# showlab/EgoVLP

Hardware: NVIDIA H100
Metric: clips/sec, 16-frame TimeSformer-B + DistilBERT + EgoNCE training step (higher is better)
Workload: dtype bf16

## Files before the change

### egovlp_b200/csrc/attention.cu

```cuda
#include <stdlib.h>

#include "common.cuh"
#include "egovlp_b200.h"

namespace egovlp {

bool space_attn_wgmma_supported(int N);
int space_attn_fwd_wgmma(const void* qkv, void* out, float* lse, float* cls_part, int B, int T, int N, int H,
                         cudaStream_t st);

namespace {

constexpr int HD = 64;
constexpr int ROW_BYTES = 128;
constexpr float LOG2E = 1.4426950408889634f;

struct Geom {
  int B, H, T, N, S, D;
  int mode;
  int PG;
  int G;
  int NP;
  int NPAD;
  int gsize;
};

__device__ __forceinline__ int row_token(const Geom& G, int g, int r) {
  if (r == G.NP) return 0;
  if (r > G.NP) return -1;
  if (G.mode == 1) return 1 + g * G.N + r;
  const int j = r / G.T, f = r - j * G.T, n = g * G.PG + j;
  return n < G.N ? 1 + f * G.N + n : -1;
}

template <int RT>
__device__ __forceinline__ int row_token_x(const Geom& G, int g, int r, int sh) {
  if (RT == 0) return row_token(G, g, r);
  if (r == G.NP) return 0;
  if (r > G.NP) return -1;
  if (RT == 1) return 1 + g * G.N + r;
  const int n = g * G.PG + (r >> sh);
  return n < G.N ? 1 + (r & ((1 << sh) - 1)) * G.N + n : -1;
}

struct Smem {
  uint32_t q, k, v, dout;
  short* gid;
  float* lse;
  float* delta;
  uint32_t stage;
  uint32_t bar;
};

__device__ __forceinline__ bool pair_valid(int gq, int gk, bool first_group) {
  if (gq >= 0) return gk == gq || gk == -2;
  if (gq == -2) return gk >= 0 || (gk == -2 && first_group);
  return false;
}

__device__ __forceinline__ void tile_window(const Geom& G, int r0, int& lo, int& hi) {
  if (r0 <= G.NP && G.NP < r0 + 16) { lo = 0; hi = G.NP; return; }
  if (r0 > G.NP) { lo = 0; hi = 0; return; }
  lo = (r0 / G.gsize) * G.gsize;
  hi = min(G.NP, ((r0 + 15) / G.gsize + 1) * G.gsize);
}
__device__ __forceinline__ bool span_active(const Geom& G, int lo, int hi, int c0, int width) {
  return (c0 < hi && c0 + width > lo) || (c0 <= G.NP && G.NP < c0 + width);
}

template <int RT = 0>
__device__ __forceinline__ void store_rows_bf16(const float (&acc)[8][4], float s0, float s1, uint32_t stage,
                                                uint8_t* stage_gen, bf16* dst, long long ld, int col0, const Geom& G,
                                                int b, int g, int r0, int lane, bool skip_cls, int sh = 0) {
  const int gq = lane >> 2, t = lane & 3;
#pragma unroll
  for (int j = 0; j < 8; ++j) {
    const uint32_t lo = pack_bf16x2(acc[j][0] * s0, acc[j][1] * s0), hi = pack_bf16x2(acc[j][2] * s1, acc[j][3] * s1);
    asm volatile("st.shared.b32 [%0], %1;" ::"r"(sw_addr(stage, gq, j) + t * 4), "r"(lo));
    asm volatile("st.shared.b32 [%0], %1;" ::"r"(sw_addr(stage, gq + 8, j) + t * 4), "r"(hi));
  }
  __syncwarp();
#pragma unroll
  for (int p = 0; p < 4; ++p) {
    const int rr = p * 4 + (lane >> 3), c = lane & 7;
    const int tok = row_token_x<RT>(G, g, r0 + rr, sh);
    if (tok > 0 || (tok == 0 && !skip_cls)) {
      const uint4 v = *reinterpret_cast<const uint4*>(stage_gen + (sw_addr(stage, rr, c) - stage));
      *reinterpret_cast<uint4*>(dst + ((long long)b * G.S + tok) * ld + col0 + c * 8) = v;
    }
  }
  __syncwarp();
}

template <int RT = 0>
__device__ __forceinline__ void store_frag_rows_bf16(const float (&acc)[8][4], float s, bf16* dst, long long ld, int col0,
                                                     const Geom& G, int b, int g, int r0, int lane, float s_hi = -1.f,
                                                     int sh = 0) {
  const float sB = s_hi >= 0.f ? s_hi : s;
  const int gq = lane >> 2, t = lane & 3;
  const int tok0 = row_token_x<RT>(G, g, r0 + gq, sh), tok1 = row_token_x<RT>(G, g, r0 + gq + 8, sh);
  bf16* p0 = dst + ((long long)b * G.S + tok0) * ld + col0 + 2 * t;
  bf16* p1 = dst + ((long long)b * G.S + tok1) * ld + col0 + 2 * t;
#pragma unroll
  for (int j = 0; j < 8; ++j) {
    if (tok0 > 0) *reinterpret_cast<uint32_t*>(p0 + 8 * j) = pack_bf16x2(acc[j][0] * s, acc[j][1] * s);
    if (tok1 > 0) *reinterpret_cast<uint32_t*>(p1 + 8 * j) = pack_bf16x2(acc[j][2] * sB, acc[j][3] * sB);
  }
}

__device__ __forceinline__ int tile_uniform_gid(const short* gid, int r0) {
  const int a = gid[r0], b = gid[r0 + 15];
  return (a >= 0 && a == b) ? a : -1;
}

__device__ __forceinline__ void decode_block(const Geom& G, int& b, int& h, int& g) {
  h = blockIdx.x % G.H;
  const int bg = blockIdx.x / G.H;
  g = bg % G.G;
  b = bg / G.G;
}

template <bool BWD, bool STAGE = !BWD, bool WAIT = true, bool GID = true>
__device__ __forceinline__ void load_group(const Geom& G, const CUtensorMap* tm_qkv, const CUtensorMap* tm_do,
                                           const bf16* qkv, const bf16* dout, int b, int h, int g, uint8_t* smem_gen,
                                           uint32_t smem_base, Smem& sm, int nwarps) {
  const int tile_bytes = G.NPAD * ROW_BYTES;
  sm.q = smem_base;
  sm.k = sm.q + tile_bytes;
  sm.v = sm.k + tile_bytes;
  sm.dout = sm.v + tile_bytes;
  uint32_t off = (BWD ? 4 : 3) * tile_bytes;
  sm.stage = smem_base + off;
  if (STAGE) off += nwarps * 16 * ROW_BYTES;
  sm.lse = reinterpret_cast<float*>(smem_gen + off);
  off += G.NPAD * 4;
  sm.delta = reinterpret_cast<float*>(smem_gen + off);
  off += G.NPAD * 4;
  sm.gid = reinterpret_cast<short*>(smem_gen + off);
  off += ((G.NPAD * 2 + 15) / 16) * 16;
  sm.bar = smem_base + off;

  const int tid = threadIdx.x;
  if (tid == 0) {
    mbar_init(sm.bar, 1);
    fence_mbar_init();
  }
  __syncthreads();
  const int ntiles = BWD ? 4 : 3;
  if (tid == 0) {
    const int rows = (G.mode == 1) ? G.N : G.T * G.PG;
    mbar_expect_tx(sm.bar, (uint32_t)(ntiles * rows * ROW_BYTES));
    const int f0 = (G.mode == 1) ? g : 0, n0 = (G.mode == 1) ? 0 : g * G.PG;
    tma_load_5d(sm.q, tm_qkv, sm.bar, 0, f0, n0, 0 * G.H + h, b);
    tma_load_5d(sm.k, tm_qkv, sm.bar, 0, f0, n0, 1 * G.H + h, b);
    tma_load_5d(sm.v, tm_qkv, sm.bar, 0, f0, n0, 2 * G.H + h, b);
    if (BWD) tma_load_5d(sm.dout, tm_do, sm.bar, 0, f0, n0, h, b);
  }
  const int pad_rows = G.NPAD - G.NP;
  for (int i = tid; i < pad_rows * 8; i += blockDim.x) {
    const int c = i & 7, rr = i >> 3;
#pragma unroll
    for (int which = 0; which < ntiles; ++which) {
      uint4 val = make_uint4(0, 0, 0, 0);
      if (rr == 0) {
        const bf16* src = (which < 3) ? qkv + (long long)b * G.S * 3 * G.D + which * G.D + h * HD
                                      : dout + (long long)b * G.S * G.D + h * HD;
        val = *reinterpret_cast<const uint4*>(src + c * 8);
      }
      *reinterpret_cast<uint4*>(smem_gen + (sw_addr(sm.q + which * tile_bytes, G.NP + rr, c) - smem_base)) = val;
    }
  }
  if (GID) {
    for (int r = tid; r < G.NPAD; r += blockDim.x) {
      short gid = -1;
      if (r == G.NP) gid = -2;
      else if (r < G.NP && row_token(G, g, r) > 0) gid = (short)(r / G.gsize);
      sm.gid[r] = gid;
    }
  }
  __syncthreads();
  if (WAIT) mbar_wait(sm.bar, 0);
}

template <int NWARPS, int MINB>
__global__ void __launch_bounds__(NWARPS * 32, MINB)
divided_attn_fwd_kernel(const __grid_constant__ CUtensorMap tm_qkv, const bf16* __restrict__ qkv,
                        bf16* __restrict__ out, float* __restrict__ lse_out, float* __restrict__ cls_part, Geom G) {
  extern __shared__ uint8_t smem_raw[];
  const uint32_t smem_base = (smem_u32(smem_raw) + 1023u) & ~1023u;
  uint8_t* smem_gen = smem_raw + (smem_base - smem_u32(smem_raw));
  int b, h, g;
  decode_block(G, b, h, g);
  Smem sm;
  load_group<false>(G, &tm_qkv, nullptr, qkv, nullptr, b, h, g, smem_gen, smem_base, sm, NWARPS);

  const int warp = threadIdx.x >> 5, lane = threadIdx.x & 31;
  const int gq = lane >> 2, t = lane & 3;
  const bool first_group = (g == 0);
  const int NT = G.NPAD / 8;
  const uint32_t stage = sm.stage + warp * 16 * ROW_BYTES;
  uint8_t* stage_gen = smem_gen + (stage - smem_base);

  for (int rt = warp; rt * 16 <= G.NP; rt += NWARPS) {
    const int r0 = rt * 16;
    int lo, hi;
    tile_window(G, r0, lo, hi);
    uint32_t qf[4][4];
#pragma unroll
    for (int kk = 0; kk < 4; ++kk) load_a_frag(sm.q, r0, kk, lane, qf[kk]);
    const int gid0 = sm.gid[r0 + gq], gid1 = sm.gid[r0 + gq + 8];
    const int ugid = tile_uniform_gid(sm.gid, r0);
    float m0 = -INFINITY, m1 = -INFINITY, l0 = 0.f, l1 = 0.f;
    float o[8][4];
#pragma unroll
    for (int j = 0; j < 8; ++j) { o[j][0] = o[j][1] = o[j][2] = o[j][3] = 0.f; }

    for (int c0 = 0; c0 < NT; c0 += 8) {
      if (!span_active(G, lo, hi, c0 * 8, 64)) continue;
      float s[8][4];
#pragma unroll
      for (int j = 0; j < 8; ++j) { s[j][0] = s[j][1] = s[j][2] = s[j][3] = 0.f; }
#pragma unroll
      for (int p = 0; p < 4; ++p) {
        const int n0 = (c0 + 2 * p) * 8;
        if (c0 + 2 * p < NT && span_active(G, lo, hi, n0, 16)) {
#pragma unroll
          for (int kk = 0; kk < 4; ++kk) {
            uint32_t bf[4];
            load_b_frag_nk(sm.k, n0, kk, lane, bf);
            mma_bf16(s[2 * p], qf[kk], bf[0], bf[1]);
            mma_bf16(s[2 * p + 1], qf[kk], bf[2], bf[3]);
          }
        }
      }
      float cm0 = -INFINITY, cm1 = -INFINITY;
#pragma unroll
      for (int j = 0; j < 8; ++j) {
        const int col = (c0 + j) * 8 + 2 * t;
        const bool inb = (c0 + j) < NT;
        const bool fast = inb && ugid >= 0 && sm.gid[(c0 + j) * 8] == ugid && sm.gid[(c0 + j) * 8 + 7] == ugid;
        if (!fast) {
          const int k0 = inb ? sm.gid[col] : -1, k1 = inb ? sm.gid[col + 1] : -1;
          s[j][0] = pair_valid(gid0, k0, first_group) ? s[j][0] : -INFINITY;
          s[j][1] = pair_valid(gid0, k1, first_group) ? s[j][1] : -INFINITY;
          s[j][2] = pair_valid(gid1, k0, first_group) ? s[j][2] : -INFINITY;
          s[j][3] = pair_valid(gid1, k1, first_group) ? s[j][3] : -INFINITY;
        }
        cm0 = fmaxf(cm0, fmaxf(s[j][0], s[j][1]));
        cm1 = fmaxf(cm1, fmaxf(s[j][2], s[j][3]));
      }
      cm0 = fmaxf(cm0, __shfl_xor_sync(0xffffffffu, cm0, 1)); cm0 = fmaxf(cm0, __shfl_xor_sync(0xffffffffu, cm0, 2));
      cm1 = fmaxf(cm1, __shfl_xor_sync(0xffffffffu, cm1, 1)); cm1 = fmaxf(cm1, __shfl_xor_sync(0xffffffffu, cm1, 2));
      const float mn0 = fmaxf(m0, cm0), mn1 = fmaxf(m1, cm1);
      const float ms0 = (mn0 == -INFINITY) ? 0.f : mn0, ms1 = (mn1 == -INFINITY) ? 0.f : mn1;
      const float a0 = exp2f((m0 - ms0) * LOG2E), a1 = exp2f((m1 - ms1) * LOG2E);
      m0 = mn0; m1 = mn1;
      l0 *= a0; l1 *= a1;
#pragma unroll
      for (int j = 0; j < 8; ++j) { o[j][0] *= a0; o[j][1] *= a0; o[j][2] *= a1; o[j][3] *= a1; }
      uint32_t pf[4][4];
#pragma unroll
      for (int j = 0; j < 8; ++j) {
        const float p0 = exp2f((s[j][0] - ms0) * LOG2E), p1 = exp2f((s[j][1] - ms0) * LOG2E);
        const float p2 = exp2f((s[j][2] - ms1) * LOG2E), p3 = exp2f((s[j][3] - ms1) * LOG2E);
        l0 += p0 + p1; l1 += p2 + p3;
        pf[j >> 1][(j & 1) * 2] = pack_bf16x2(p0, p1);
        pf[j >> 1][(j & 1) * 2 + 1] = pack_bf16x2(p2, p3);
      }
#pragma unroll
      for (int kk = 0; kk < 4; ++kk) {
        const int k0 = (c0 + 2 * kk) * 8;
        if (c0 + 2 * kk < NT && span_active(G, lo, hi, k0, 16)) {
#pragma unroll
// ... 448 lines not shown
#pragma unroll
    for (int dp = 0; dp < 4; ++dp) {
      uint32_t bf[4];
      ldsm_x4_t(vb + fo.a[dp], bf);
      mma_bf16(o[2 * dp], pf[p], bf[0], bf[1]);
      mma_bf16(o[2 * dp + 1], pf[p], bf[2], bf[3]);
    }
  }
}

template <bool TIME, int NWARPS, int MINB>
__global__ void __launch_bounds__(NWARPS * 32, MINB)
fast_attn_fwd_kernel(const __grid_constant__ CUtensorMap tm_qkv, const bf16* __restrict__ qkv, bf16* __restrict__ out,
                     float* __restrict__ lse_out, float* __restrict__ cls_part, Geom G, int sh) {
  extern __shared__ uint8_t smem_raw[];
  const uint32_t smem_base = (smem_u32(smem_raw) + 1023u) & ~1023u;
  uint8_t* smem_gen = smem_raw + (smem_base - smem_u32(smem_raw));
  int b, h, g;
  decode_block(G, b, h, g);
  Smem sm;
  load_group<false, !TIME, true, false>(G, &tm_qkv, nullptr, qkv, nullptr, b, h, g, smem_gen, smem_base, sm, NWARPS);
  constexpr int RT = TIME ? 2 : 1;

  const int warp = threadIdx.x >> 5, lane = threadIdx.x & 31;
  const int gq = lane >> 2, t = lane & 3;
  FastCtx c;
  c.NP = G.NP; c.NPAD = G.NPAD; c.sh = sh; c.first_group = (g == 0);
  c.valid_keys = TIME ? min(G.PG, G.N - g * G.PG) * G.T : G.NP;
  const FragOff fo = make_frag_off(lane);
  const uint32_t stage = sm.stage + warp * 16 * ROW_BYTES;
  uint8_t* stage_gen = smem_gen + (stage - smem_base);

  for (int it = warp;; it += NWARPS) {
    int r0, part;
    if (!work_item<TIME, NWARPS>(c, it, r0, part)) break;
    const int rowA = r0 + gq, rowB = rowA + 8;
    uint32_t qf[4][4];
#pragma unroll
    for (int kk = 0; kk < 4; ++kk) ldsm_x4(sm.q + r0 * ROW_BYTES + fo.a[kk], qf[kk]);
    float m0 = -INFINITY, m1 = -INFINITY, l0 = 0.f, l1 = 0.f;
    float o[8][4];
#pragma unroll
    for (int j = 0; j < 8; ++j) { o[j][0] = o[j][1] = o[j][2] = o[j][3] = 0.f; }
    Chunk ch;
#pragma unroll 1
    for (int ci = 0; get_chunk<TIME, NWARPS, 4>(c, G.T, r0, part, ci, ch); ++ci) {
      switch (ch.np) {
        case 4: fwd_chunk<TIME, 4>(c, sm, fo, ch, qf, rowA, rowB, t, m0, m1, l0, l1, o); break;
        case 3: fwd_chunk<TIME, 3>(c, sm, fo, ch, qf, rowA, rowB, t, m0, m1, l0, l1, o); break;
        case 2: fwd_chunk<TIME, 2>(c, sm, fo, ch, qf, rowA, rowB, t, m0, m1, l0, l1, o); break;
        default: fwd_chunk<TIME, 1>(c, sm, fo, ch, qf, rowA, rowB, t, m0, m1, l0, l1, o); break;
      }
    }
    l0 += __shfl_xor_sync(0xffffffffu, l0, 1); l0 += __shfl_xor_sync(0xffffffffu, l0, 2);
    l1 += __shfl_xor_sync(0xffffffffu, l1, 1); l1 += __shfl_xor_sync(0xffffffffu, l1, 2);
    {
      const int rc = c.NP - r0;
      if (rc >= 0 && rc < 16 && (rc & 7) == gq) {
        const bool hi_half = rc >= 8;
        constexpr int PARTS = TIME ? NWARPS : 1;
        float* dst = cls_part + ((((long long)(b * G.H + h)) * G.G + g) * PARTS + max(part, 0)) * 66;
#pragma unroll
        for (int j = 0; j < 8; ++j) {
          dst[j * 8 + 2 * t] = hi_half ? o[j][2] : o[j][0];
          dst[j * 8 + 2 * t + 1] = hi_half ? o[j][3] : o[j][1];
        }
        if (t == 0) { dst[64] = hi_half ? m1 : m0; dst[65] = hi_half ? l1 : l0; }
      }
    }
    if (part >= 0) continue;
    const float i0 = l0 > 0.f ? 1.f / l0 : 0.f, i1 = l1 > 0.f ? 1.f / l1 : 0.f;
    if (t == 0) {
      const int tok0 = row_token_x<RT>(G, g, rowA, sh), tok1 = row_token_x<RT>(G, g, rowB, sh);
      if (tok0 > 0) lse_out[((long long)(b * G.H + h)) * G.S + tok0] = m0 + logf(l0);
      if (tok1 > 0) lse_out[((long long)(b * G.H + h)) * G.S + tok1] = m1 + logf(l1);
    }
    if (TIME) store_frag_rows_bf16<RT>(o, i0, out, G.D, h * HD, G, b, g, r0, lane, i1, sh);
    else store_rows_bf16<RT>(o, i0, i1, stage, stage_gen, out, G.D, h * HD, G, b, g, r0, lane, true, sh);
  }
}

template <bool TIME, int NPR>
__device__ __forceinline__ void bwd_q_chunk(const FastCtx& c, const Smem& sm, const FragOff& fo, const Chunk& ch, int r0,
                                            int rowA, int rowB, int t, float ls0, float ls1, float de0, float de1,
                                            float (&dq)[8][4]) {
  float s[2 * NPR][4], dp[2 * NPR][4];
#pragma unroll
  for (int j = 0; j < 2 * NPR; ++j) { s[j][0] = s[j][1] = s[j][2] = s[j][3] = 0.f; dp[j][0] = dp[j][1] = dp[j][2] = dp[j][3] = 0.f; }
#pragma unroll
  for (int kk = 0; kk < 4; ++kk) {
    uint32_t aq[4], ad[4];
    ldsm_x4(sm.q + r0 * ROW_BYTES + fo.a[kk], aq);
    ldsm_x4(sm.dout + r0 * ROW_BYTES + fo.a[kk], ad);
#pragma unroll
    for (int p = 0; p < NPR; ++p) {
      uint32_t bf[4];
      ldsm_x4(sm.k + ch.base[p] * ROW_BYTES + fo.b[kk], bf);
      mma_bf16(s[2 * p], aq, bf[0], bf[1]);
      mma_bf16(s[2 * p + 1], aq, bf[2], bf[3]);
      ldsm_x4(sm.v + ch.base[p] * ROW_BYTES + fo.b[kk], bf);
      mma_bf16(dp[2 * p], ad, bf[0], bf[1]);
      mma_bf16(dp[2 * p + 1], ad, bf[2], bf[3]);
    }
  }
  uint32_t dsf[NPR][4];
  const f32x2 sc = pk2(LOG2E, LOG2E), nl0 = pk2(-ls0, -ls0), nl1 = pk2(-ls1, -ls1);
  const f32x2 nd0 = pk2(-de0, -de0), nd1 = pk2(-de1, -de1);
#pragma unroll
  for (int p = 0; p < NPR; ++p) {
    const bool masked = ch.mask & (1u << p);
#pragma unroll
    for (int jj = 0; jj < 2; ++jj) {
      const int j = 2 * p + jj, col = ch.base[p] + 8 * jj + 2 * t;
      if (masked) {
        if (TIME && ch.base[p] == c.NP && r0 < c.NP) {
          const bool kc = jj == 0 && t == 0;
          s[j][0] = kc ? s[j][0] : -INFINITY; s[j][1] = -INFINITY;
          s[j][2] = kc ? s[j][2] : -INFINITY; s[j][3] = -INFINITY;
        } else if (TIME && r0 >= c.NP && ch.base[p] < c.NP) {
          const bool cq = rowA == c.NP;
          s[j][0] = (cq && col < c.valid_keys) ? s[j][0] : -INFINITY;
          s[j][1] = (cq && col + 1 < c.valid_keys) ? s[j][1] : -INFINITY;
          s[j][2] = -INFINITY; s[j][3] = -INFINITY;
        } else {
          s[j][0] = fast_valid<TIME>(c, rowA, col) ? s[j][0] : -INFINITY;
          s[j][1] = fast_valid<TIME>(c, rowA, col + 1) ? s[j][1] : -INFINITY;
          s[j][2] = fast_valid<TIME>(c, rowB, col) ? s[j][2] : -INFINITY;
          s[j][3] = fast_valid<TIME>(c, rowB, col + 1) ? s[j][3] : -INFINITY;
        }
      }
      float e0, e1, e2, e3;
      up2(fma2(pk2(s[j][0], s[j][1]), sc, nl0), e0, e1);
      up2(fma2(pk2(s[j][2], s[j][3]), sc, nl1), e2, e3);
      float d0, d1, d2, d3;
      up2(mul2(pk2(exp2f(e0), exp2f(e1)), add2(pk2(dp[j][0], dp[j][1]), nd0)), d0, d1);
      up2(mul2(pk2(exp2f(e2), exp2f(e3)), add2(pk2(dp[j][2], dp[j][3]), nd1)), d2, d3);
      dsf[p][jj * 2] = pack_bf16x2(d0, d1);
      dsf[p][jj * 2 + 1] = pack_bf16x2(d2, d3);
    }
  }
#pragma unroll
  for (int p = 0; p < NPR; ++p) {
    const uint32_t kb = sm.k + ch.base[p] * ROW_BYTES;
#pragma unroll
    for (int dpi = 0; dpi < 4; ++dpi) {
      uint32_t bf[4];
      ldsm_x4_t(kb + fo.a[dpi], bf);
      mma_bf16(dq[2 * dpi], dsf[p], bf[0], bf[1]);
      mma_bf16(dq[2 * dpi + 1], dsf[p], bf[2], bf[3]);
    }
  }
}

template <bool TIME, int NPR>
__device__ __forceinline__ void bwd_k_chunk(const FastCtx& c, const Smem& sm, const FragOff& fo, const Chunk& ch, int k0r,
                                            int keyA, int keyB, int t, float (&dk)[8][4], float (&dv)[8][4]) {
  float st[2 * NPR][4], dpt[2 * NPR][4];
#pragma unroll
  for (int j = 0; j < 2 * NPR; ++j) { st[j][0] = st[j][1] = st[j][2] = st[j][3] = 0.f; dpt[j][0] = dpt[j][1] = dpt[j][2] = dpt[j][3] = 0.f; }
#pragma unroll
  for (int kk = 0; kk < 4; ++kk) {
    uint32_t ak[4], av[4];
    ldsm_x4(sm.k + k0r * ROW_BYTES + fo.a[kk], ak);
    ldsm_x4(sm.v + k0r * ROW_BYTES + fo.a[kk], av);
#pragma unroll
    for (int p = 0; p < NPR; ++p) {
      uint32_t bf[4];
      ldsm_x4(sm.q + ch.base[p] * ROW_BYTES + fo.b[kk], bf);
      mma_bf16(st[2 * p], ak, bf[0], bf[1]);
      mma_bf16(st[2 * p + 1], ak, bf[2], bf[3]);
      ldsm_x4(sm.dout + ch.base[p] * ROW_BYTES + fo.b[kk], bf);
      mma_bf16(dpt[2 * p], av, bf[0], bf[1]);
      mma_bf16(dpt[2 * p + 1], av, bf[2], bf[3]);
    }
  }
  uint32_t pf[NPR][4], dsf[NPR][4];
  const f32x2 sc = pk2(LOG2E, LOG2E);
#pragma unroll
  for (int p = 0; p < NPR; ++p) {
    const bool masked = ch.mask & (1u << p);
#pragma unroll
    for (int jj = 0; jj < 2; ++jj) {
      const int j = 2 * p + jj, col = ch.base[p] + 8 * jj + 2 * t;
      if (masked) {
        if (TIME && ch.base[p] == c.NP && k0r < c.NP) {
          const bool qc = jj == 0 && t == 0;
          st[j][0] = (qc && keyA < c.valid_keys) ? st[j][0] : -INFINITY; st[j][1] = -INFINITY;
          st[j][2] = (qc && keyB < c.valid_keys) ? st[j][2] : -INFINITY; st[j][3] = -INFINITY;
        } else if (TIME && k0r >= c.NP && ch.base[p] < c.NP) {
          const bool ck = keyA == c.NP;
          st[j][0] = ck ? st[j][0] : -INFINITY; st[j][1] = ck ? st[j][1] : -INFINITY;
          st[j][2] = -INFINITY; st[j][3] = -INFINITY;
        } else {
          st[j][0] = fast_valid<TIME>(c, col, keyA) ? st[j][0] : -INFINITY;
          st[j][1] = fast_valid<TIME>(c, col + 1, keyA) ? st[j][1] : -INFINITY;
          st[j][2] = fast_valid<TIME>(c, col, keyB) ? st[j][2] : -INFINITY;
          st[j][3] = fast_valid<TIME>(c, col + 1, keyB) ? st[j][3] : -INFINITY;
        }
      }
      const float2 lq = *reinterpret_cast<const float2*>(sm.lse + col);
      const float2 dq2 = *reinterpret_cast<const float2*>(sm.delta + col);
      const f32x2 nl = pk2(-lq.x, -lq.y), nd = pk2(-dq2.x, -dq2.y);
      float e0, e1, e2, e3;
      up2(fma2(pk2(st[j][0], st[j][1]), sc, nl), e0, e1);
      up2(fma2(pk2(st[j][2], st[j][3]), sc, nl), e2, e3);
      const float p0 = exp2f(e0), p1 = exp2f(e1), p2 = exp2f(e2), p3 = exp2f(e3);
      pf[p][jj * 2] = pack_bf16x2(p0, p1);
      pf[p][jj * 2 + 1] = pack_bf16x2(p2, p3);
      float d0, d1, d2, d3;
      up2(mul2(pk2(p0, p1), add2(pk2(dpt[j][0], dpt[j][1]), nd)), d0, d1);
      up2(mul2(pk2(p2, p3), add2(pk2(dpt[j][2], dpt[j][3]), nd)), d2, d3);
      dsf[p][jj * 2] = pack_bf16x2(d0, d1);
      dsf[p][jj * 2 + 1] = pack_bf16x2(d2, d3);
    }
  }
#pragma unroll
  for (int p = 0; p < NPR; ++p) {
    const uint32_t qb = sm.q + ch.base[p] * ROW_BYTES, db = sm.dout + ch.base[p] * ROW_BYTES;
#pragma unroll
    for (int dpi = 0; dpi < 4; ++dpi) {
      uint32_t bf[4];
      ldsm_x4_t(db + fo.a[dpi], bf);
      mma_bf16(dv[2 * dpi], pf[p], bf[0], bf[1]);
      mma_bf16(dv[2 * dpi + 1], pf[p], bf[2], bf[3]);
      ldsm_x4_t(qb + fo.a[dpi], bf);
      mma_bf16(dk[2 * dpi], dsf[p], bf[0], bf[1]);
      mma_bf16(dk[2 * dpi + 1], dsf[p], bf[2], bf[3]);
    }
  }
}

template <bool TIME, int NWARPS, int MINB, bool DET>
__global__ void __launch_bounds__(NWARPS * 32, MINB)
fast_attn_bwd_kernel(const __grid_constant__ CUtensorMap tm_qkv, const __grid_constant__ CUtensorMap tm_do,
                     const bf16* __restrict__ qkv, const bf16* __restrict__ out, const bf16* __restrict__ dout,
                     const float* __restrict__ lse_in, bf16* __restrict__ dqkv, float* __restrict__ dcls, float q_scale,
                     Geom G, int sh) {
  extern __shared__ uint8_t smem_raw[];
  const uint32_t smem_base = (smem_u32(smem_raw) + 1023u) & ~1023u;
  uint8_t* smem_gen = smem_raw + (smem_base - smem_u32(smem_raw));
  int b, h, g;
  decode_block(G, b, h, g);
  Smem sm;
  load_group<true, false, false, false>(G, &tm_qkv, &tm_do, qkv, dout, b, h, g, smem_gen, smem_base, sm, NWARPS);
  constexpr int RT = TIME ? 2 : 1;

  const int warp = threadIdx.x >> 5, lane = threadIdx.x & 31;
  const int gq = lane >> 2, t = lane & 3;
  FastCtx c;
  c.NP = G.NP; c.NPAD = G.NPAD; c.sh = sh; c.first_group = (g == 0);
  c.valid_keys = TIME ? min(G.PG, G.N - g * G.PG) * G.T : G.NP;
  const FragOff fo = make_frag_off(lane);

  constexpr int P0_ROWS = NWARPS * 4;
  constexpr int P0_MAX = (256 + P0_ROWS - 1) / P0_ROWS;
  constexpr int P0_N = TIME ? 128 / P0_ROWS : P0_MAX;
  uint4 o_pre[P0_N];
  float l_pre[P0_N];
  int t_pre[P0_N];
#pragma unroll
  for (int i = 0; i < P0_N; ++i) {
    const int r = warp * 4 + (lane >> 3) + i * P0_ROWS;
    const int tok = r < G.NPAD ? row_token_x<RT>(G, g, r, sh) : -1;
    t_pre[i] = tok;
    const int tc = max(tok, 0);
    o_pre[i] = __ldg(reinterpret_cast<const uint4*>(out + ((long long)b * G.S + tc) * G.D + h * HD + (lane & 7) * 8));
    l_pre[i] = __ldg(lse_in + ((long long)(b * G.H + h)) * G.S + tc);
  }
  mbar_wait(sm.bar, 0);
#pragma unroll
  for (int i = 0; i < P0_N; ++i) {
    const int r = warp * 4 + (lane >> 3) + i * P0_ROWS;
    if (r >= G.NPAD) break;
    const int tok = t_pre[i], cc = lane & 7;
    float d = 0.f;
    if (tok >= 0) {
      const uint4 ov = o_pre[i];
      const uint4 dv = *reinterpret_cast<const uint4*>(smem_gen + (sw_addr(sm.dout, r, cc) - smem_base));
      const uint32_t ou[4] = {ov.x, ov.y, ov.z, ov.w}, du[4] = {dv.x, dv.y, dv.z, dv.w};
#pragma unroll
      for (int i = 0; i < 4; ++i) {
        const float2 a = unpack_bf16x2(ou[i]), bb = unpack_bf16x2(du[i]);
        d += a.x * bb.x + a.y * bb.y;
      }
    }
    d += __shfl_xor_sync(0xffffffffu, d, 1); d += __shfl_xor_sync(0xffffffffu, d, 2); d += __shfl_xor_sync(0xffffffffu, d, 4);
    if (cc == 0) {
      sm.delta[r] = d;
      sm.lse[r] = tok >= 0 ? l_pre[i] * LOG2E : 0.f;
    }
  }
  __syncthreads();

  for (int it = warp;; it += NWARPS) {
    int r0, part;
    if (!work_item<TIME, NWARPS>(c, it, r0, part)) break;
    const int rowA = r0 + gq, rowB = rowA + 8;
    const float ls0 = sm.lse[rowA], ls1 = sm.lse[rowB], de0 = sm.delta[rowA], de1 = sm.delta[rowB];
    float dq[8][4];
#pragma unroll
    for (int j = 0; j < 8; ++j) { dq[j][0] = dq[j][1] = dq[j][2] = dq[j][3] = 0.f; }
    Chunk ch;
#pragma unroll 1
    for (int ci = 0; get_chunk<TIME, NWARPS, 2>(c, G.T, r0, part, ci, ch); ++ci) {
      if (ch.np == 2) bwd_q_chunk<TIME, 2>(c, sm, fo, ch, r0, rowA, rowB, t, ls0, ls1, de0, de1, dq);
      else bwd_q_chunk<TIME, 1>(c, sm, fo, ch, r0, rowA, rowB, t, ls0, ls1, de0, de1, dq);
    }
    {
      const int rc = c.NP - r0;
      if (rc >= 0 && rc < 16 && (rc & 7) == gq) {
        const bool hi_half = rc >= 8;
#pragma unroll
        for (int j = 0; j < 8; ++j) {
          cls_grad_put<DET>(dcls, G, b, h, g, TIME ? NWARPS : 1, max(part, 0), 0, j * 8 + 2 * t, hi_half ? dq[j][2] : dq[j][0]);
          cls_grad_put<DET>(dcls, G, b, h, g, TIME ? NWARPS : 1, max(part, 0), 0, j * 8 + 2 * t + 1, hi_half ? dq[j][3] : dq[j][1]);
        }
      }
    }
    if (part < 0) store_frag_rows_bf16<RT>(dq, q_scale, dqkv, 3 * G.D, h * HD, G, b, g, r0, lane, -1.f, sh);
  }

  for (int it = warp;; it += NWARPS) {
    int k0r, part;
    if (!work_item<TIME, NWARPS>(c, it, k0r, part)) break;
    const int keyA = k0r + gq, keyB = keyA + 8;
    float dk[8][4], dv[8][4];
#pragma unroll
    for (int j = 0; j < 8; ++j) { dk[j][0] = dk[j][1] = dk[j][2] = dk[j][3] = 0.f; dv[j][0] = dv[j][1] = dv[j][2] = dv[j][3] = 0.f; }
    Chunk ch;
#pragma unroll 1
    for (int ci = 0; get_chunk<TIME, NWARPS, 2>(c, G.T, k0r, part, ci, ch); ++ci) {
      if (ch.np == 2) bwd_k_chunk<TIME, 2>(c, sm, fo, ch, k0r, keyA, keyB, t, dk, dv);
      else bwd_k_chunk<TIME, 1>(c, sm, fo, ch, k0r, keyA, keyB, t, dk, dv);
    }
    {
      const int rc = c.NP - k0r;
      if (rc >= 0 && rc < 16 && (rc & 7) == gq) {
        const bool hi_half = rc >= 8;
#pragma unroll
        for (int j = 0; j < 8; ++j) {
          cls_grad_put<DET>(dcls, G, b, h, g, TIME ? NWARPS : 1, max(part, 0), 1, j * 8 + 2 * t, hi_half ? dk[j][2] : dk[j][0]);
          cls_grad_put<DET>(dcls, G, b, h, g, TIME ? NWARPS : 1, max(part, 0), 1, j * 8 + 2 * t + 1, hi_half ? dk[j][3] : dk[j][1]);
          cls_grad_put<DET>(dcls, G, b, h, g, TIME ? NWARPS : 1, max(part, 0), 2, j * 8 + 2 * t, hi_half ? dv[j][2] : dv[j][0]);
          cls_grad_put<DET>(dcls, G, b, h, g, TIME ? NWARPS : 1, max(part, 0), 2, j * 8 + 2 * t + 1, hi_half ? dv[j][3] : dv[j][1]);
        }
      }
    }
    if (part < 0) {
      store_frag_rows_bf16<RT>(dk, 1.f, dqkv, 3 * G.D, G.D + h * HD, G, b, g, k0r, lane, -1.f, sh);
      store_frag_rows_bf16<RT>(dv, 1.f, dqkv, 3 * G.D, 2 * G.D + h * HD, G, b, g, k0r, lane, -1.f, sh);
    }
  }
}

inline bool force_generic() {
  const char* e = getenv("EGOVLP_ATTN_GENERIC");
  return e && e[0] == '1';
}
inline bool time_fast_ok(const Geom& G) { return G.mode == 0 && (G.T == 4 || G.T == 8 || G.T == 16) && G.NP == 112; }
inline int time_shift(const Geom& G) { return G.T == 16 ? 4 : G.T == 8 ? 3 : 2; }

int make_geom(Geom& G, int B, int T, int N, int H, int mode) {
  G.B = B; G.H = H; G.T = T; G.N = N; G.S = 1 + T * N; G.D = H * HD; G.mode = mode;
  if (mode == 1) {
    G.PG = N; G.G = T; G.NP = N; G.gsize = N;
  } else {
    G.PG = (T <= 16 && 16 % T == 0) ? min(N, 112 / T) : min(N, 127 / T);
    if (G.PG < 1) return EGOVLP_ERR_UNSUPPORTED;
    G.G = (N + G.PG - 1) / G.PG; G.NP = G.PG * T; G.gsize = T;
  }
  G.NPAD = (G.NP + 1 + 15) / 16 * 16;
  if (G.NPAD > 256 || (mode == 1 ? N : max(T, G.PG)) > 256) return EGOVLP_ERR_UNSUPPORTED;
  return EGOVLP_OK;
}

int make_group_tmap(CUtensorMap* tm, const void* base, const Geom& G, int ncolblk) {
  const uint64_t W = (uint64_t)ncolblk * HD;
  const uint64_t dims[5] = {HD, (uint64_t)G.T, (uint64_t)G.N, (uint64_t)ncolblk, (uint64_t)G.B};
  const uint64_t strides[5] = {1, (uint64_t)G.N * W, W, HD, (uint64_t)G.S * W};
  const uint32_t box[5] = {HD, (uint32_t)(G.mode == 1 ? 1 : G.T), (uint32_t)(G.mode == 1 ? G.N : G.PG), 1, 1};
  return make_tmap_nd_bf16(tm, reinterpret_cast<const bf16*>(base) + W, 5, dims, strides, box, true);
}

size_t attn_smem_bytes(const Geom& G, bool bwd, int nwarps, bool staging = true) {
  return (size_t)(bwd ? 4 : 3) * G.NPAD * ROW_BYTES + ((bwd || !staging) ? 0 : nwarps * 16 * ROW_BYTES) + 2 * G.NPAD * 4 +
         ((G.NPAD * 2 + 15) / 16) * 16 + 16 + 1024;
}


}
}

using namespace egovlp;

extern "C" long long egovlp_divided_attn_workspace_floats(int B, int T, int N, int H, int mode) {
  Geom G;
  if (make_geom(G, B, T, N, H, mode)) return -1;
  return (long long)B * H * G.G * 4 * 66;
}

extern "C" int egovlp_divided_attn_fwd(const void* qkv, void* out, float* lse, float* cls_part, int B, int T, int N,
                                       int H, int mode, void* stream) {
  EGOVLP_CHECK_ARG(qkv && out && lse && cls_part, "divided_attn_fwd: null pointer");
  EGOVLP_CHECK_ARG(B > 0 && T > 0 && N > 0 && H > 0 && (mode == 0 || mode == 1), "divided_attn_fwd: bad shape");
  Geom G;
  if (make_geom(G, B, T, N, H, mode)) { set_last_error("divided_attn: unsupported geometry T=%d N=%d", T, N); return EGOVLP_ERR_UNSUPPORTED; }
  CUtensorMap tm;
  int rc = make_group_tmap(&tm, qkv, G, 3 * H);
  if (rc) return rc;
  cudaStream_t st = reinterpret_cast<cudaStream_t>(stream);
  const bf16* q = reinterpret_cast<const bf16*>(qkv);
  bf16* o = reinterpret_cast<bf16*>(out);
  const int grid = B * H * G.G;
#define LAUNCH_FWD(KERN, W, ...)                                                                              \
  do {                                                                                                        \
    const size_t smem = attn_smem_bytes(G, false, W, generic || mode == 1);                                   \
    EGOVLP_CHECK_CUDA(cudaFuncSetAttribute(KERN, cudaFuncAttributeMaxDynamicSharedMemorySize, (int)smem));    \
    KERN<<<grid, W * 32, smem, st>>>(tm, q, o, lse, cls_part, G, ##__VA_ARGS__);                              \
  } while (0)
  const bool generic = force_generic() || (mode == 0 && !time_fast_ok(G));
  if (!generic && mode == 1 && space_attn_wgmma_supported(N)) {
    rc = space_attn_fwd_wgmma(qkv, out, lse, cls_part, B, T, N, H, st);
    if (rc) return rc;
  } else if (generic) {
    if (G.NPAD > 128) LAUNCH_FWD((divided_attn_fwd_kernel<7, 2>), 7);
    else LAUNCH_FWD((divided_attn_fwd_kernel<4, 3>), 4);
  } else if (mode == 1) {
    if (G.NPAD > 128) LAUNCH_FWD((fast_attn_fwd_kernel<false, 7, 2>), 7, 0);
    else LAUNCH_FWD((fast_attn_fwd_kernel<false, 4, 3>), 4, 0);
  } else {
    LAUNCH_FWD((fast_attn_fwd_kernel<true, 4, 4>), 4, time_shift(G));
  }
#undef LAUNCH_FWD
  EGOVLP_CHECK_LAUNCH();
  const int BH = B * H;
  const int parts = (!generic && mode == 0) ? 4 : 1;
  cls_merge_kernel<<<(BH + 3) / 4, 128, 0, st>>>(cls_part, o, lse, BH, H, G.G * parts, G.S, G.D);
  EGOVLP_CHECK_LAUNCH();
  return EGOVLP_OK;
}

static int divided_attn_bwd_impl(const void* qkv, const void* out, const void* dout, const float* lse, void* dqkv,
                                 float* dcls_ws, int B, int T, int N, int H, int mode, float q_scale, bool det,
                                 void* stream) {
  EGOVLP_CHECK_ARG(qkv && out && dout && lse && dqkv && dcls_ws, "divided_attn_bwd: null pointer");
  EGOVLP_CHECK_ARG(B > 0 && T > 0 && N > 0 && H > 0 && (mode == 0 || mode == 1), "divided_attn_bwd: bad shape");
  Geom G;
  if (make_geom(G, B, T, N, H, mode)) { set_last_error("divided_attn: unsupported geometry T=%d N=%d", T, N); return EGOVLP_ERR_UNSUPPORTED; }
  CUtensorMap tmq, tmd;
  int rc = make_group_tmap(&tmq, qkv, G, 3 * H);
  if (rc) return rc;
  rc = make_group_tmap(&tmd, dout, G, H);
  if (rc) return rc;
  cudaStream_t st = reinterpret_cast<cudaStream_t>(stream);
  if (!det) EGOVLP_CHECK_CUDA(cudaMemsetAsync(dcls_ws, 0, (size_t)B * H * 3 * HD * sizeof(float), st));
  const bf16* q = reinterpret_cast<const bf16*>(qkv);
  const bf16* o = reinterpret_cast<const bf16*>(out);
  const bf16* d_o = reinterpret_cast<const bf16*>(dout);
  bf16* dq = reinterpret_cast<bf16*>(dqkv);
  const int grid = B * H * G.G;
#define LAUNCH_BWD(KERN, W, ...)                                                                              \
  do {                                                                                                        \
    const size_t smem = attn_smem_bytes(G, true, W);                                                          \
    EGOVLP_CHECK_CUDA(cudaFuncSetAttribute(KERN, cudaFuncAttributeMaxDynamicSharedMemorySize, (int)smem));    \
    KERN<<<grid, W * 32, smem, st>>>(tmq, tmd, q, o, d_o, lse, dq, dcls_ws, q_scale, G, ##__VA_ARGS__);       \
  } while (0)
  const bool generic = (!det && force_generic()) || (mode == 0 && !time_fast_ok(G));
  int slots = 1;
  if (det) {
    slots = G.G * (generic || mode == 1 ? 1 : 4);
    if (generic) {
      if (G.NPAD > 128) LAUNCH_BWD((divided_attn_bwd_kernel<7, 2, true>), 7);
      else LAUNCH_BWD((divided_attn_bwd_kernel<4, 3, true>), 4);
    } else if (mode == 1) {
      if (G.NPAD > 128) LAUNCH_BWD((fast_attn_bwd_kernel<false, 7, 2, true>), 7, 0);
      else LAUNCH_BWD((fast_attn_bwd_kernel<false, 4, 3, true>), 4, 0);
    } else {
      LAUNCH_BWD((fast_attn_bwd_kernel<true, 4, 3, true>), 4, time_shift(G));
    }
  } else if (generic) {
    if (G.NPAD > 128) LAUNCH_BWD((divided_attn_bwd_kernel<7, 2, false>), 7);
    else LAUNCH_BWD((divided_attn_bwd_kernel<4, 3, false>), 4);
  } else if (mode == 1) {
    if (G.NPAD > 128) LAUNCH_BWD((fast_attn_bwd_kernel<false, 7, 2, false>), 7, 0);
    else LAUNCH_BWD((fast_attn_bwd_kernel<false, 4, 3, false>), 4, 0);
  } else {
    const char* we = getenv("EGOVLP_ATTN_TIME_BWD_WARPS");
    const bool w8 = we && we[0] == '8';
    if (w8) LAUNCH_BWD((fast_attn_bwd_kernel<true, 8, 2, false>), 8, time_shift(G));
    else LAUNCH_BWD((fast_attn_bwd_kernel<true, 4, 3, false>), 4, time_shift(G));
  }
#undef LAUNCH_BWD
  EGOVLP_CHECK_LAUNCH();
  const int n = B * H * 3 * HD;
  cls_grad_finalize_kernel<<<(n + 255) / 256, 256, 0, st>>>(dcls_ws, reinterpret_cast<bf16*>(dqkv), B, H, G.S, G.D, q_scale,
                                                             slots);
  EGOVLP_CHECK_LAUNCH();
  return EGOVLP_OK;
}

extern "C" int egovlp_divided_attn_bwd(const void* qkv, const void* out, const void* dout, const float* lse,
                                       void* dqkv, float* dcls_ws, int B, int T, int N, int H, int mode,
                                       float q_scale, void* stream) {
  return divided_attn_bwd_impl(qkv, out, dout, lse, dqkv, dcls_ws, B, T, N, H, mode, q_scale, false, stream);
}

extern "C" long long egovlp_divided_attn_bwd_det_workspace_floats(int B, int T, int N, int H, int mode) {
  Geom G;
  if (B <= 0 || H <= 0 || (mode != 0 && mode != 1) || make_geom(G, B, T, N, H, mode)) return -1;
  const int parts = (mode == 0 && time_fast_ok(G)) ? 4 : 1;
  return (long long)B * H * G.G * parts * 3 * HD;
}

extern "C" int egovlp_divided_attn_bwd_det(const void* qkv, const void* out, const void* dout, const float* lse,
                                           void* dqkv, float* dcls_ws, int B, int T, int N, int H, int mode,
                                           float q_scale, void* stream) {
  return divided_attn_bwd_impl(qkv, out, dout, lse, dqkv, dcls_ws, B, T, N, H, mode, q_scale, true, stream);
}
```

Baseline: 184.0.

## Add persistent space-attention backward kernel that reuses stored dS for dQ

Adds a dedicated persistent backward kernel for spatial attention (mode 1). One warp handles each 16-row key tile, and the whole group fits in one block. During the dK/dV pass it writes the dS tile to shared memory, and dQ is then computed from that stored dS instead of recomputing scores. The kernel also loops over groups with TMA prefetch of the next group's Q/V/dO and K, overlapping loads with compute. It trades a large shared-memory footprint, one block per SM and extra barriers for less recomputation and less load latency.

```diff
diff --git a/egovlp_b200/csrc/attention.cu b/egovlp_b200/csrc/attention.cu
--- a/egovlp_b200/csrc/attention.cu
+++ b/egovlp_b200/csrc/attention.cu
@@ -113,12 +113,13 @@
   return (a >= 0 && a == b) ? a : -1;
 }
 
-__device__ __forceinline__ void decode_block(const Geom& G, int& b, int& h, int& g) {
-  h = blockIdx.x % G.H;
-  const int bg = blockIdx.x / G.H;
+__device__ __forceinline__ void decode_block(const Geom& G, unsigned blk, int& b, int& h, int& g) {
+  h = blk % G.H;
+  const int bg = blk / G.H;
   g = bg % G.G;
   b = bg / G.G;
 }
+__device__ __forceinline__ void decode_block(const Geom& G, int& b, int& h, int& g) { decode_block(G, blockIdx.x, b, h, g); }
 
 template <bool BWD, bool STAGE = !BWD, bool WAIT = true, bool GID = true>
 __device__ __forceinline__ void load_group(const Geom& G, const CUtensorMap* tm_qkv, const CUtensorMap* tm_do,
@@ -873,9 +874,10 @@
   }
 }
 
-template <bool TIME, int NPR>
+template <bool TIME, int NPR, bool DS_OUT = false>
 __device__ __forceinline__ void bwd_k_chunk(const FastCtx& c, const Smem& sm, const FragOff& fo, const Chunk& ch, int k0r,
-                                            int keyA, int keyB, int t, float (&dk)[8][4], float (&dv)[8][4]) {
+                                            int keyA, int keyB, int t, float (&dk)[8][4], float (&dv)[8][4],
+                                            uint32_t ds_t = 0, uint32_t ds_ld = 0) {
   float st[2 * NPR][4], dpt[2 * NPR][4];
 #pragma unroll
   for (int j = 0; j < 2 * NPR; ++j) { st[j][0] = st[j][1] = st[j][2] = st[j][3] = 0.f; dpt[j][0] = dpt[j][1] = dpt[j][2] = dpt[j][3] = 0.f; }
@@ -933,6 +935,10 @@
       up2(mul2(pk2(p2, p3), add2(pk2(dpt[j][2], dpt[j][3]), nd)), d2, d3);
       dsf[p][jj * 2] = pack_bf16x2(d0, d1);
       dsf[p][jj * 2 + 1] = pack_bf16x2(d2, d3);
+      if (DS_OUT) {
+        asm volatile("st.shared.b32 [%0], %1;" ::"r"(ds_t + keyA * ds_ld + col * 2), "r"(dsf[p][jj * 2]));
+        asm volatile("st.shared.b32 [%0], %1;" ::"r"(ds_t + keyB * ds_ld + col * 2), "r"(dsf[p][jj * 2 + 1]));
+      }
     }
   }
 #pragma unroll
@@ -1074,6 +1080,193 @@
   }
 }
 
+constexpr int SPACE_BWD_MAX_NPAD = 224;
+
+__host__ __device__ __forceinline__ uint32_t space_bwd_ds_ld(int NPAD) { return (uint32_t)NPAD * 2 + 16; }
+
+size_t space_bwd_smem_bytes(const Geom& G) {
+  return (size_t)4 * G.NPAD * ROW_BYTES + (size_t)G.NPAD * space_bwd_ds_ld(G.NPAD) + 2 * G.NPAD * 4 + 16 + 1024;
+}
+
+template <bool DET>
+__global__ void __launch_bounds__(SPACE_BWD_MAX_NPAD / 16 * 32, 1)
+space_attn_bwd_kernel(const __grid_constant__ CUtensorMap tm_qkv, const __grid_constant__ CUtensorMap tm_do,
+                      const bf16* __restrict__ qkv, const bf16* __restrict__ out, const bf16* __restrict__ dout,
+                      const float* __restrict__ lse_in, bf16* __restrict__ dqkv, float* __restrict__ dcls, float q_scale,
+                      Geom G) {
+  extern __shared__ uint8_t smem_raw[];
+  const uint32_t smem_base = (smem_u32(smem_raw) + 1023u) & ~1023u;
+  uint8_t* smem_gen = smem_raw + (smem_base - smem_u32(smem_raw));
+  const int NP = G.NP, NPAD = G.NPAD;
+  const uint32_t tile_bytes = NPAD * ROW_BYTES, ds_ld = space_bwd_ds_ld(NPAD);
+  Smem sm;
+  sm.q = smem_base;
+  sm.k = sm.q + tile_bytes;
+  sm.v = sm.k + tile_bytes;
+  sm.dout = sm.v + tile_bytes;
+  const uint32_t ds_t = smem_base + 4 * tile_bytes;
+  uint32_t off = 4 * tile_bytes + NPAD * ds_ld;
+  sm.lse = reinterpret_cast<float*>(smem_gen + off);
+  off += NPAD * 4;
+  sm.delta = reinterpret_cast<float*>(smem_gen + off);
+  off += NPAD * 4;
+  const uint32_t bar_qvd = smem_base + off, bar_k = bar_qvd + 8;
+
+  const int tid = threadIdx.x, warp = tid >> 5, lane = tid & 31;
+  const int gq = lane >> 2, t = lane & 3;
+  const int ngroups = G.B * G.H * G.G;
+  auto load_qvd = [&](int blk) {
+    int b, h, g;
+    decode_block(G, blk, b, h, g);
+    mbar_expect_tx(bar_qvd, (uint32_t)(3 * G.N * ROW_BYTES));
+    tma_load_5d(sm.q, &tm_qkv, bar_qvd, 0, g, 0, h, b);
+    tma_load_5d(sm.v, &tm_qkv, bar_qvd, 0, g, 0, 2 * G.H + h, b);
+    tma_load_5d(sm.dout, &tm_do, bar_qvd, 0, g, 0, h, b);
+  };
+  auto load_k = [&](int blk) {
+    int b, h, g;
+    decode_block(G, blk, b, h, g);
+    mbar_expect_tx(bar_k, (uint32_t)(G.N * ROW_BYTES));
+    tma_load_5d(sm.k, &tm_qkv, bar_k, 0, g, 0, G.H + h, b);
+  };
+
+  if (tid == 0) {
+    mbar_init(bar_qvd, 1);
+    mbar_init(bar_k, 1);
+    fence_mbar_init();
+  }
+  const int pad_chunks = (NPAD - NP - 1) * 8;
+  for (int i = tid; i < 4 * pad_chunks; i += blockDim.x) {
+    const int which = i / pad_chunks, rem = i - which * pad_chunks;
+    *reinterpret_cast<uint4*>(smem_gen + (sw_addr(sm.q + which * tile_bytes, NP + 1 + (rem >> 3), rem & 7) - smem_base)) =
+        make_uint4(0, 0, 0, 0);
+  }
+  __syncthreads();
+  if (tid == 0) {
+    load_qvd(blockIdx.x);
+    load_k(blockIdx.x);
+  }
+
+  FastCtx c;
+  c.NP = NP; c.NPAD = NPAD; c.sh = 0; c.valid_keys = NP;
+  const FragOff fo = make_frag_off(lane);
+  const int r0 = warp * 16;
+  const int rowA = r0 + gq, rowB = rowA + 8;
+  const int rc = NP - r0;
+  const bool cls_lane = rc >= 0 && rc < 16 && (rc & 7) == gq, cls_hi = rc >= 8;
+  uint32_t phase = 0;
+  for (int blk = blockIdx.x; blk < ngroups; blk += gridDim.x, phase ^= 1) {
+    int b, h, g;
+    decode_block(G, blk, b, h, g);
+    c.first_group = (g == 0);
+    const int next = blk + gridDim.x;
+    if (tid < 32) {
+      const int which = tid >> 3, cc = tid & 7;
+      const bf16* src = (which < 3) ? qkv + (long long)b * G.S * 3 * G.D + which * G.D + h * HD
+                                    : dout + (long long)b * G.S * G.D + h * HD;
+      *reinterpret_cast<uint4*>(smem_gen + (sw_addr(sm.q + which * tile_bytes, NP, cc) - smem_base)) =
+          *reinterpret_cast<const uint4*>(src + cc * 8);
+    }
+    uint4 o_pre[4];
+    float l_pre[4];
+    int t_pre[4];
+#pragma unroll
+    for (int i = 0; i < 4; ++i) {
+      const int r = warp * 4 + (lane >> 3) + i * (NPAD / 4);
+      const int tok = row_token_x<1>(G, g, r, 0);
+      t_pre[i] = tok;
+      const int tc = max(tok, 0);
+      o_pre[i] = __ldg(reinterpret_cast<const uint4*>(out + ((long long)b * G.S + tc) * G.D + h * HD + (lane & 7) * 8));
+      l_pre[i] = __ldg(lse_in + ((long long)(b * G.H + h)) * G.S + tc);
+    }
+    __syncthreads();
+    mbar_wait_nocall(bar_qvd, phase);
+#pragma unroll
+    for (int i = 0; i < 4; ++i) {
+      const int r = warp * 4 + (lane >> 3) + i * (NPAD / 4);
+      const int tok = t_pre[i], cc = lane & 7;
+      float d = 0.f;
+      if (tok >= 0) {
+        const uint4 dv = *reinterpret_cast<const uint4*>(smem_gen + (sw_addr(sm.dout, r, cc) - smem_base));
+        const uint32_t ou[4] = {o_pre[i].x, o_pre[i].y, o_pre[i].z, o_pre[i].w}, du[4] = {dv.x, dv.y, dv.z, dv.w};
+#pragma unroll
+        for (int k = 0; k < 4; ++k) {
+          const float2 a = unpack_bf16x2(ou[k]), bb = unpack_bf16x2(du[k]);
+          d += a.x * bb.x + a.y * bb.y;
+        }
+      }
+      d += __shfl_xor_sync(0xffffffffu, d, 1); d += __shfl_xor_sync(0xffffffffu, d, 2); d += __shfl_xor_sync(0xffffffffu, d, 4);
+      if (cc == 0) {
+        sm.delta[r] = d;
+        sm.lse[r] = tok >= 0 ? l_pre[i] * LOG2E : 0.f;
+      }
+    }
+    mbar_wait_nocall(bar_k, phase);
+    __syncthreads();
+
+    {
+      float dk[8][4], dv[8][4];
+#pragma unroll
+      for (int j = 0; j < 8; ++j) { dk[j][0] = dk[j][1] = dk[j][2] = dk[j][3] = 0.f; dv[j][0] = dv[j][1] = dv[j][2] = dv[j][3] = 0.f; }
+      Chunk ch;
+#pragma unroll 1
+      for (int ci = 0; get_chunk<false, 1, 2>(c, G.T, r0, -1, ci, ch); ++ci) {
+        if (ch.np == 2) bwd_k_chunk<false, 2, true>(c, sm, fo, ch, r0, rowA, rowB, t, dk, dv, ds_t, ds_ld);
+        else bwd_k_chunk<false, 1, true>(c, sm, fo, ch, r0, rowA, rowB, t, dk, dv, ds_t, ds_ld);
+      }
+      if (cls_lane) {
+#pragma unroll
+        for (int j = 0; j < 8; ++j) {
+          cls_grad_put<DET>(dcls, G, b, h, g, 1, 0, 1, j * 8 + 2 * t, cls_hi ? dk[j][2] : dk[j][0]);
+          cls_grad_put<DET>(dcls, G, b, h, g, 1, 0, 1, j * 8 + 2 * t + 1, cls_hi ? dk[j][3] : dk[j][1]);
+          cls_grad_put<DET>(dcls, G, b, h, g, 1, 0, 2, j * 8 + 2 * t, cls_hi ? dv[j][2] : dv[j][0]);
+          cls_grad_put<DET>(dcls, G, b, h, g, 1, 0, 2, j * 8 + 2 * t + 1, cls_hi ? dv[j][3] : dv[j][1]);
+        }
+      }
+      store_frag_rows_bf16<1>(dk, 1.f, dqkv, 3 * G.D, G.D + h * HD, G, b, g, r0, lane);
+      store_frag_rows_bf16<1>(dv, 1.f, dqkv, 3 * G.D, 2 * G.D + h * HD, G, b, g, r0, lane);
+    }
+    __syncthreads();
+    if (tid == 0 && next < ngroups) {
+      fence_proxy_async_smem();
+      load_qvd(next);
+    }
+
+    {
+      float dq[8][4];
+#pragma unroll
+      for (int j = 0; j < 8; ++j) { dq[j][0] = dq[j][1] = dq[j][2] = dq[j][3] = 0.f; }
+      const uint32_t a_row = ds_t + ((lane & 7) + (lane >> 4) * 8) * ds_ld + (r0 + ((lane >> 3) & 1) * 8) * 2;
+#pragma unroll 1
+      for (int kp = 0; kp < NPAD; kp += 16) {
+        uint32_t af[4];
+        ldsm_x4_t(a_row + kp * ds_ld, af);
+        const uint32_t kb = sm.k + kp * ROW_BYTES;
+#pragma unroll
+        for (int dpi = 0; dpi < 4; ++dpi) {
+          uint32_t bf[4];
+          ldsm_x4_t(kb + fo.a[dpi], bf);
+          mma_bf16(dq[2 * dpi], af, bf[0], bf[1]);
+          mma_bf16(dq[2 * dpi + 1], af, bf[2], bf[3]);
+        }
+      }
+      if (cls_lane) {
+#pragma unroll
+        for (int j = 0; j < 8; ++j) {
+          cls_grad_put<DET>(dcls, G, b, h, g, 1, 0, 0, j * 8 + 2 * t, cls_hi ? dq[j][2] : dq[j][0]);
+          cls_grad_put<DET>(dcls, G, b, h, g, 1, 0, 0, j * 8 + 2 * t + 1, cls_hi ? dq[j][3] : dq[j][1]);
+        }
+      }
+      store_frag_rows_bf16<1>(dq, q_scale, dqkv, 3 * G.D, h * HD, G, b, g, r0, lane);
+    }
+    __syncthreads();
+    if (tid == 0 && next < ngroups) {
+      fence_proxy_async_smem();
+      load_k(next);
+    }
+  }
+}
+
 inline bool force_generic() {
   const char* e = getenv("EGOVLP_ATTN_GENERIC");
   return e && e[0] == '1';
@@ -1101,6 +1294,20 @@
   const uint64_t strides[5] = {1, (uint64_t)G.N * W, W, HD, (uint64_t)G.S * W};
   const uint32_t box[5] = {HD, (uint32_t)(G.mode == 1 ? 1 : G.T), (uint32_t)(G.mode == 1 ? G.N : G.PG), 1, 1};
   return make_tmap_nd_bf16(tm, reinterpret_cast<const bf16*>(base) + W, 5, dims, strides, box, true);
+}
+
+template <bool DET>
+int launch_space_bwd(const Geom& G, const CUtensorMap& tmq, const CUtensorMap& tmd, const bf16* qkv, const bf16* out,
+                     const bf16* dout, const float* lse, bf16* dqkv, float* dcls, float q_scale, cudaStream_t st) {
+  const size_t smem = space_bwd_smem_bytes(G);
+  const int threads = G.NPAD / 16 * 32;
+  EGOVLP_CHECK_CUDA(cudaFuncSetAttribute(space_attn_bwd_kernel<DET>, cudaFuncAttributeMaxDynamicSharedMemorySize, (int)smem));
+  int per_sm = 0;
+  EGOVLP_CHECK_CUDA(cudaOccupancyMaxActiveBlocksPerMultiprocessor(&per_sm, space_attn_bwd_kernel<DET>, threads, smem));
+  const long long groups = (long long)G.B * G.H * G.G;
+  const int grid = (int)std::min<long long>(groups, (long long)std::max(per_sm, 1) * num_sms());
+  space_attn_bwd_kernel<DET><<<grid, threads, smem, st>>>(tmq, tmd, qkv, out, dout, lse, dqkv, dcls, q_scale, G);
+  return EGOVLP_OK;
 }
 
 size_t attn_smem_bytes(const Geom& G, bool bwd, int nwarps, bool staging = true) {
@@ -1194,8 +1401,8 @@
       if (G.NPAD > 128) LAUNCH_BWD((divided_attn_bwd_kernel<7, 2, true>), 7);
       else LAUNCH_BWD((divided_attn_bwd_kernel<4, 3, true>), 4);
     } else if (mode == 1) {
-      if (G.NPAD > 128) LAUNCH_BWD((fast_attn_bwd_kernel<false, 7, 2, true>), 7, 0);
-      else LAUNCH_BWD((fast_attn_bwd_kernel<false, 4, 3, true>), 4, 0);
+      if (G.NPAD <= SPACE_BWD_MAX_NPAD) rc = launch_space_bwd<true>(G, tmq, tmd, q, o, d_o, lse, dq, dcls_ws, q_scale, st);
+      else LAUNCH_BWD((fast_attn_bwd_kernel<false, 7, 2, true>), 7, 0);
     } else {
       LAUNCH_BWD((fast_attn_bwd_kernel<true, 4, 3, true>), 4, time_shift(G));
     }
@@ -1203,8 +1410,8 @@
     if (G.NPAD > 128) LAUNCH_BWD((divided_attn_bwd_kernel<7, 2, false>), 7);
     else LAUNCH_BWD((divided_attn_bwd_kernel<4, 3, false>), 4);
   } else if (mode == 1) {
-    if (G.NPAD > 128) LAUNCH_BWD((fast_attn_bwd_kernel<false, 7, 2, false>), 7, 0);
-    else LAUNCH_BWD((fast_attn_bwd_kernel<false, 4, 3, false>), 4, 0);
+    if (G.NPAD <= SPACE_BWD_MAX_NPAD) rc = launch_space_bwd<false>(G, tmq, tmd, q, o, d_o, lse, dq, dcls_ws, q_scale, st);
+    else LAUNCH_BWD((fast_attn_bwd_kernel<false, 7, 2, false>), 7, 0);
   } else {
     const char* we = getenv("EGOVLP_ATTN_TIME_BWD_WARPS");
     const bool w8 = we && we[0] == '8';
@@ -1212,6 +1419,7 @@
     else LAUNCH_BWD((fast_attn_bwd_kernel<true, 4, 3, false>), 4, time_shift(G));
   }
 #undef LAUNCH_BWD
+  if (rc) return rc;
   EGOVLP_CHECK_LAUNCH();
   const int n = B * H * 3 * HD;
   cls_grad_finalize_kernel<<<(n + 255) / 256, 256, 0, st>>>(dcls_ws, reinterpret_cast<bf16*>(dqkv), B, H, G.S, G.D, q_scale,
```

Result: faster. 186.4, median of 6 (+1.3%).
